# VITA-Group/LightGaussian

Hardware: NVIDIA H100
Metric: training views/sec at 3M Gaussians 1080p (higher is better)
Workload: dtype f32

## Files before the change

lightgaussian_b200/csrc/lgr_blend.cuh:

```cuda
#pragma once

namespace {

constexpr int BL_CH = 32;
constexpr int BL_STAGES = 4;
constexpr int BL_REC = 12;
constexpr int BL_THREADS = 288;
constexpr uint32_t BL_END = 0xffffffffu;
constexpr int BL_FLUSH = 16;
constexpr int BL_ROW = 33;

__device__ __forceinline__ void mbar_arrive(uint64_t* bar)
{
    asm volatile("mbarrier.arrive.shared::cta.b64 _, [%0];" ::"r"(smem_u32(bar)) : "memory");
}
__device__ __forceinline__ void mbar_wait_ring(uint64_t* bar, uint32_t parity)
{
    for (uint32_t spin = 0; !mbar_try_wait(bar, parity); ++spin)
        if (spin > (1u << 26)) {
            printf("lgrast: blend ring barrier timed out (block %d warp %d)\n", (int)blockIdx.x, (int)(threadIdx.x >> 5));
            __trap();
        }
}
template <int N>
// ... 31 lines not shown

constexpr int KB_ZERO_BYTES = 5760;

struct KbackZeroArgs {
    int P, nrest;
    const int* radii;
    const float* acc;
    int* idx;
    int* counter;
    float* d_xyz; float* d_dc; float* d_rest; float* d_scaling; float* d_rotation; float* d_opacity; float* dL_dmeans2D;
};

__device__ __forceinline__ void bulk_zero(float* dst, size_t floats, const void* zero_page)
{
    size_t bytes = floats * 4;
    char* p = reinterpret_cast<char*>(dst);
    while (bytes) {
        const uint32_t n = (uint32_t)(bytes < (size_t)KB_ZERO_BYTES ? bytes : (size_t)KB_ZERO_BYTES);
        bulk_s2g(p, zero_page, n);
        p += n;
        bytes -= n;
    }
}


__device__ __forceinline__ void tile_zero_rows(const KbackZeroArgs& z, int tile, int tiles, const void* zero_page)
{
    const int G = ((z.P + tiles - 1) / tiles + 3) & ~3;
    const long long first = (long long)tile * G;
    if (first >= z.P) return;
    const int n = (int)min((long long)G, z.P - first), nb = n & ~3;
    if (nb) {
        bulk_zero(z.d_rest + (size_t)first * z.nrest, (size_t)nb * z.nrest, zero_page);
        bulk_zero(z.d_dc + (size_t)first * 3, (size_t)nb * 3, zero_page);
        bulk_zero(z.d_xyz + (size_t)first * 3, (size_t)nb * 3, zero_page);
        bulk_zero(z.d_scaling + (size_t)first * 3, (size_t)nb * 3, zero_page);
        bulk_zero(z.d_rotation + (size_t)first * 4, (size_t)nb * 4, zero_page);
        bulk_zero(z.d_opacity + (size_t)first, (size_t)nb, zero_page);
        bulk_zero(z.dL_dmeans2D + (size_t)first * 3, (size_t)nb * 3, zero_page);
        bulk_commit();
    }
    for (long long i = first + nb; i < first + n; i++) {
        for (int k = 0; k < z.nrest; k++) z.d_rest[(size_t)i * z.nrest + k] = 0.f;
        for (int k = 0; k < 3; k++) {
            z.d_dc[(size_t)i * 3 + k] = 0.f; z.d_xyz[(size_t)i * 3 + k] = 0.f; z.d_scaling[(size_t)i * 3 + k] = 0.f; z.dL_dmeans2D[(size_t)i * 3 + k] = 0.f;
        }
        for (int k = 0; k < 4; k++) z.d_rotation[(size_t)i * 4 + k] = 0.f;
        z.d_opacity[(size_t)i] = 0.f;
    }
}

struct BlendRing {
    float rec[BL_STAGES][BL_CH * BL_REC];
    uint64_t full[BL_STAGES];
    uint64_t empty[BL_STAGES];
    uint32_t count[BL_STAGES];
    int live;
    unsigned tile_max;
};

__device__ __forceinline__ void ring_init(BlendRing& r, int consumers)
{
    if (threadIdx.x == 0) {
#pragma unroll
        for (int s = 0; s < BL_STAGES; s++) {
            mbar_init(&r.full[s], 1);
            mbar_init(&r.empty[s], consumers);
        }
        r.live = consumers;
        r.tile_max = 0;
        fence_mbar_init();
    }
    __syncthreads();
}

template <bool COUNT, bool STORE, bool PERM = false>
__global__ void __launch_bounds__(BL_THREADS)
blend_forward_ring_kernel(const uint2* __restrict__ ranges, const uint32_t* __restrict__ point_list, int W, int H, int tiles_x,
                          const float2* __restrict__ means2D, const float4* __restrict__ conic_opacity, const float4* __restrict__ rgb,
                          const float* __restrict__ bg, float* __restrict__ final_T, uint32_t* __restrict__ n_contrib,
                          float* __restrict__ out_color, int* __restrict__ count, float* __restrict__ rec_out, const int* __restrict__ header,
                          const uint32_t* __restrict__ perm = nullptr)
{
    if (header[HDR_OVERFLOW]) return;
    __shared__ __align__(128) BlendRing ring;
    const int warp = threadIdx.x >> 5, lane = threadIdx.x & 31;
    const int tile = blockIdx.x;
    const uint2 range = ranges[tile];
    ring_init(ring, 8);

    if (warp == 8) {
        for (uint32_t c = 0;; c++) {
            const int s = c % BL_STAGES;
            const uint32_t ph = (c / BL_STAGES) & 1u;
            mbar_wait_ring(&ring.empty[s], ph ^ 1u);
            if (STORE) {
                if (lane == 0) bulk_wait_read<BL_STAGES - 1>();
                __syncwarp();
            }
            const uint32_t pos0 = range.x + c * BL_CH;
            const int live = *reinterpret_cast<volatile int*>(&ring.live);
            if (pos0 >= range.y || live <= 0) {
                if (lane == 0) {
                    ring.count[s] = BL_END;
                    mbar_arrive(&ring.full[s]);
                }
                break;
            }
            const uint32_t n = min((uint32_t)BL_CH, range.y - pos0);
            if ((uint32_t)lane < n) {
                const uint32_t id = point_list[pos0 + lane];
                const float2 xy = means2D[id];
                const float4 co = conic_opacity[id];
                const float4 col = rgb[id];
                float4* r4 = reinterpret_cast<float4*>(&ring.rec[s][lane * BL_REC]);
                r4[0] = make_float4(xy.x, xy.y, co.x, co.y);
                r4[1] = make_float4(co.z, co.w, col.x, col.y);
                r4[2] = make_float4(col.z, __uint_as_float(id), PERM ? __uint_as_float(perm[pos0 + lane]) : 0.f, 0.f);
            }
            if (lane == 0) ring.count[s] = n;
            if (STORE) fence_async_smem();
            __syncwarp();
            if (lane == 0) {
                if (STORE) {
                    bulk_s2g(rec_out + (size_t)pos0 * BL_REC, &ring.rec[s][0], n * (uint32_t)(BL_REC * 4));
                    bulk_commit();
                }
                mbar_arrive(&ring.full[s]);
            }
        }
        if (STORE && lane == 0) bulk_wait_all();
        return;
    }

    const int tx = tile % tiles_x, ty = tile / tiles_x;
    const int sx0 = tx * LGR_TILE + (warp & 1) * 8, sy0 = ty * LGR_TILE + (warp >> 1) * 4;
    const int px = sx0 + (lane & 7), py = sy0 + (lane >> 3);
    const bool inside = px < W && py < H;
    float pxf = (float)px, pyf = (float)py;
    const float rx0 = (float)sx0, rx1 = (float)min(sx0 + 7, W - 1), ry0 = (float)sy0, ry1 = (float)min(sy0 + 3, H - 1);

    float T = inside ? 1.0f : -1.0f;
    float C0 = 0.f, C1 = 0.f, C2 = 0.f;
    uint32_t last = 0;
    bool warp_done = __all_sync(FULL, T < 0.f);
    if (warp_done && lane == 0) atomicSub(&ring.live, 1);

    for (uint32_t c = 0;; c++) {
        const int s = c % BL_STAGES;
        const uint32_t ph = (c / BL_STAGES) & 1u;
        mbar_wait_ring(&ring.full[s], ph);
        const uint32_t n = ring.count[s];
        if (n == BL_END) break;
        if (!warp_done) {
            const float* stage = &ring.rec[s][0];
            bool keep = false;
            if ((uint32_t)lane < n) {
                const float4 q0 = *reinterpret_cast<const float4*>(stage + lane * BL_REC);
                const float4 q1 = *reinterpret_cast<const float4*>(stage + lane * BL_REC + 4);
                keep = !subtile_cull2(q0.x, q0.y, q0.z, q0.w, q1.x, q1.y, rx0, rx1, ry0, ry1);
            }
            unsigned mask = __ballot_sync(FULL, keep);
            const uint32_t pos_base = c * BL_CH + 1u;
            while (mask) {
                const int j = __ffs(mask) - 1;
                mask &= mask - 1;
                const float* r = stage + j * BL_REC;
                const float4 q0 = *reinterpret_cast<const float4*>(r);
                const float4 q1 = *reinterpret_cast<const float4*>(r + 4);
                const float dx = LGR_SUB(q0.x, pxf), dy = LGR_SUB(q0.y, pyf);
                const float power = lgr::pair_power(dx, dy, q0.z, q0.w, q1.x);
                bool contrib = false;
                if (!(power > 0.0f)) {
                    const float alpha = fminf(0.99f, LGR_MUL(q1.y, expf(power)));
                    if (!(alpha < 1.0f / 255.0f)) {
                        const float test_T = LGR_MUL(T, LGR_SUB(1.0f, alpha));
                        if (test_T < 0.0001f) {
                            T = -fabsf(T);
                        } else {
                            const float b = r[8];
                            C0 = LGR_FMA(T, LGR_MUL(alpha, q1.z), C0);
                            C1 = LGR_FMA(T, LGR_MUL(alpha, q1.w), C1);
                            C2 = LGR_FMA(T, LGR_MUL(alpha, b), C2);
                            T = test_T;
                            last = pos_base + (uint32_t)j;
                            contrib = true;
                        }
                    }
                }
                if (COUNT) {
                    const unsigned cm = __ballot_sync(FULL, contrib);
                    if (cm != 0 && lane == 0) atomicAdd(&count[__float_as_uint(r[9])], __popc(cm));
                }
                if (__all_sync(FULL, T < 0.f)) break;
            }
            warp_done = __all_sync(FULL, T < 0.f);
            if (warp_done && lane == 0) atomicSub(&ring.live, 1);
        }
        __syncwarp();
        if (lane == 0) mbar_arrive(&ring.empty[s]);
    }
    if (inside) {
        const size_t pix = (size_t)py * W + px;
        const size_t plane = (size_t)H * W;
        const float Tf = fabsf(T);
        final_T[pix] = Tf;
        n_contrib[pix] = last;
        out_color[pix] = LGR_FMA(bg[0], Tf, C0);
        out_color[plane + pix] = LGR_FMA(bg[1], Tf, C1);
        out_color[2 * plane + pix] = LGR_FMA(bg[2], Tf, C2);
    }
}

struct BlendBackWarp {
    float w[BL_FLUSH][BL_ROW];
    float g[BL_FLUSH][BL_ROW];
    float mid[BL_FLUSH], mgx[BL_FLUSH], mgy[BL_FLUSH];
    float4 d[32];
};

struct BlendDetStage {
    float c[BL_STAGES][8][BL_CH * DET_ROW];
    uint32_t mask[BL_STAGES][8];
};

__host__ __device__ __forceinline__ size_t det_partial_offset(size_t Rn)
{
    return (Rn * 4 + 255) / 256 * 256 + (Rn * 48 + 255) / 256 * 256;
}
__host__ __device__ __forceinline__ size_t det_reached_offset(size_t Rn)
{
    return det_partial_offset(Rn) + (Rn * DET_ROW * 4 + 255) / 256 * 256;
}
__host__ __device__ __forceinline__ size_t det_ids_offset(size_t Rn)
{
    return det_reached_offset(Rn) + ((Rn + 31) / 32 * 4 + 255) / 256 * 256;
}

template <bool DET = false>
__device__ __forceinline__ void back_flush(const BlendBackWarp& bw, int nbuf, int lane, float ox, float oy, float* __restrict__ acc)
{
    __syncwarp();
    const int p = lane & 15, h = lane >> 4;
    float c0 = 0.f, c1 = 0.f, c2 = 0.f, s0 = 0.f, mx = 0.f, my = 0.f, mxx = 0.f, mxy = 0.f, myy = 0.f;
    const float* wr = &bw.w[p][16 * h];
    const float* gr = &bw.g[p][16 * h];
    const float4* dr = &bw.d[16 * h];
#pragma unroll
    for (int i = 0; i < 16; i++) {
        const float w = wr[i], g = gr[i];
        const float4 d = dr[i];
        const float xl = (float)(i & 7), yl = (float)(i >> 3);
        c0 = fmaf(w, d.x, c0);
        c1 = fmaf(w, d.y, c1);
        c2 = fmaf(w, d.z, c2);
        s0 += g;
        mx = fmaf(g, xl, mx);
        my = fmaf(g, yl, my);
        mxx = fmaf(g, xl * xl, mxx);
        mxy = fmaf(g, xl * yl, mxy);
        myy = fmaf(g, yl * yl, myy);
    }
    const float X = bw.mgx[p] - ox, Y = bw.mgy[p] - (oy + 2.0f * (float)h);
    float s1x = fmaf(X, s0, -mx), s1y = fmaf(Y, s0, -my);
    float s2xx = fmaf(X, fmaf(X, s0, -2.0f * mx), mxx);
    float s2xy = fmaf(X, fmaf(Y, s0, -my), fmaf(-Y, mx, mxy));
    float s2yy = fmaf(Y, fmaf(Y, s0, -2.0f * my), myy);
    c0 += __shfl_xor_sync(FULL, c0, 16);
    c1 += __shfl_xor_sync(FULL, c1, 16);
    c2 += __shfl_xor_sync(FULL, c2, 16);
    s0 += __shfl_xor_sync(FULL, s0, 16);
    s1x += __shfl_xor_sync(FULL, s1x, 16);
    s1y += __shfl_xor_sync(FULL, s1y, 16);
    s2xx += __shfl_xor_sync(FULL, s2xx, 16);
    s2xy += __shfl_xor_sync(FULL, s2xy, 16);
    s2yy += __shfl_xor_sync(FULL, s2yy, 16);
    if (DET && p < nbuf) {
        float* row = acc + __float_as_uint(bw.mid[p]) * DET_ROW;
        if (h == 0) {
            row[0] = c0; row[1] = c1; row[2] = c2; row[3] = s0; row[4] = s1x;
        } else {
            row[5] = s1y; row[6] = s2xx; row[7] = s2xy; row[8] = s2yy;
        }
    } else if (p < nbuf) {
        float* rec = acc + (size_t)__float_as_uint(bw.mid[p]) * ACC_STRIDE;
        if (h == 0) {
            red_add_v4(rec, c0, c1, c2, s0);
        } else {
            red_add_v4(rec + 4, s1x, s1y, s2xx, s2xy);
            atomicAdd(rec + 8, s2yy);
        }
    }
    __syncwarp();
}

constexpr size_t BL_DET_BYTES = (sizeof(BlendDetStage) + 127) / 128 * 128;

constexpr size_t blend_back_smem_bytes(bool zero_rows = false, bool det = false)
{
    return (sizeof(BlendRing) + 127) / 128 * 128 + (8 * sizeof(BlendBackWarp) + 127) / 128 * 128 + (det ? BL_DET_BYTES : 0) +
           (zero_rows ? (size_t)KB_ZERO_BYTES : 0);
}

template <bool DET = false>
__global__ void __launch_bounds__(BL_THREADS)
blend_backward_ring_kernel(const uint2* __restrict__ ranges, const char* __restrict__ binning_blob, const int* __restrict__ header, int W, int H,
                           int tiles_x, const float* __restrict__ bg, const float* __restrict__ final_T, const uint32_t* __restrict__ n_contrib,
                           const float* __restrict__ dL_dpix, float* __restrict__ acc, KbackZeroArgs zero)
{
    extern __shared__ __align__(128) unsigned char blend_dyn_smem[];
    BlendRing& ring = *reinterpret_cast<BlendRing*>(blend_dyn_smem);
    BlendBackWarp* warps = reinterpret_cast<BlendBackWarp*>(blend_dyn_smem + ((sizeof(BlendRing) + 127) / 128) * 128);
    unsigned char* behind_warps = reinterpret_cast<unsigned char*>(warps) + (8 * sizeof(BlendBackWarp) + 127) / 128 * 128;
    BlendDetStage* det = reinterpret_cast<BlendDetStage*>(behind_warps);
    const int warp = threadIdx.x >> 5, lane = threadIdx.x & 31;
    const int tile = blockIdx.x;
    const uint2 range = ranges[tile];
    float* zero_page = reinterpret_cast<float*>(behind_warps + (DET ? BL_DET_BYTES : 0));
    const bool zero_rows = zero.P > 0;
    if (zero_rows) {
        for (int k = threadIdx.x; k < KB_ZERO_BYTES / 4; k += BL_THREADS) zero_page[k] = 0.f;
        fence_async_smem();
    }
    ring_init(ring, 8);
    if (zero_rows && threadIdx.x == 8 * 32) tile_zero_rows(zero, tile, gridDim.x, zero_page);

    const int tx = tile % tiles_x, ty = tile / tiles_x;
    const int sx0 = tx * LGR_TILE + (warp & 1) * 8, sy0 = ty * LGR_TILE + (warp >> 1) * 4;
    const int px = sx0 + (lane & 7), py = sy0 + (lane >> 3);
    const bool inside = warp < 8 && px < W && py < H;
    const size_t pix = (size_t)py * W + px;
    const size_t plane = (size_t)H * W;
    const uint32_t last = inside ? n_contrib[pix] : 0u;
    const uint32_t warp_max = __reduce_max_sync(FULL, last);
    if (lane == 0 && warp_max) atomicMax(&ring.tile_max, warp_max);
    __syncthreads();
    const uint32_t tile_max = ring.tile_max;
    if (tile_max == 0 || (DET && header[HDR_DET] != 1)) {
        if (zero_rows && threadIdx.x == 8 * 32) bulk_wait_all();
        return;
    }
    const uint32_t nchunks = (tile_max + BL_CH - 1) / BL_CH;

    if (DET && warp == 8) {
        const size_t Rn = (size_t)max(header[HDR_CAPACITY], 1);
        const float* rec_in = reinterpret_cast<const float*>(binning_blob + (Rn * 4 + 255) / 256 * 256);
        float* partial = reinterpret_cast<float*>(const_cast<char*>(binning_blob) + det_partial_offset(Rn));
        uint32_t* reached = reinterpret_cast<uint32_t*>(const_cast<char*>(binning_blob) + det_reached_offset(Rn));
        for (uint32_t i = 0; i < nchunks + BL_STAGES; i++) {
            const int s = i % BL_STAGES;
            const uint32_t ph = (i / BL_STAGES) & 1u;
            if (i >= BL_STAGES) {
                mbar_wait_ring(&ring.empty[s], ph ^ 1u);
                const uint32_t b = nchunks - 1 - (i - BL_STAGES);
                const uint32_t n = min((uint32_t)BL_CH, tile_max - b * BL_CH);
                if ((uint32_t)lane < n) {
                    const uint32_t u = __float_as_uint(ring.rec[s][lane * BL_REC + 10]);
                    float v[DET_ROW];
#pragma unroll
                    for (int k = 0; k < DET_ROW; k++) v[k] = 0.f;
#pragma unroll
                    for (int w = 0; w < 8; w++) {
                        if ((det->mask[s][w] >> lane) & 1u) {
                            const float* c = &det->c[s][w][lane * DET_ROW];
#pragma unroll
                            for (int k = 0; k < DET_ROW; k++) v[k] += c[k];
                        }
                    }
                    if (u < Rn) {
#pragma unroll
                        for (int k = 0; k < DET_ROW; k++) partial[(size_t)u * DET_ROW + k] = v[k];
                        atomicOr(&reached[u >> 5], 1u << (u & 31));
                    }
                }
                __syncwarp();
            }
            if (i >= nchunks) continue;
            if (lane == 0) {
                if (i < BL_STAGES) mbar_wait_ring(&ring.empty[s], ph ^ 1u);
                const uint32_t b = nchunks - 1 - i;
                const uint32_t n = min((uint32_t)BL_CH, tile_max - b * BL_CH);
                const uint32_t bytes = n * (uint32_t)(BL_REC * 4);
                mbar_expect_tx(&ring.full[s], bytes);
                bulk_g2s(&ring.rec[s][0], rec_in + ((size_t)range.x + (size_t)b * BL_CH) * BL_REC, bytes, &ring.full[s]);
            }
            __syncwarp();
        }
        if (zero_rows && lane == 0) bulk_wait_all();
        return;
    }
    if (warp == 8) {
        if (lane == 0) {
            const size_t Rn = (size_t)max(header[HDR_CAPACITY], 1);
            const float* rec_in = reinterpret_cast<const float*>(binning_blob + (Rn * 4 + 255) / 256 * 256);
            for (uint32_t i = 0; i < nchunks; i++) {
                const uint32_t b = nchunks - 1 - i;
                const int s = i % BL_STAGES;
                const uint32_t ph = (i / BL_STAGES) & 1u;
                mbar_wait_ring(&ring.empty[s], ph ^ 1u);
                const uint32_t n = min((uint32_t)BL_CH, tile_max - b * BL_CH);
                const uint32_t bytes = n * (uint32_t)(BL_REC * 4);
                mbar_expect_tx(&ring.full[s], bytes);
                bulk_g2s(&ring.rec[s][0], rec_in + ((size_t)range.x + (size_t)b * BL_CH) * BL_REC, bytes, &ring.full[s]);
            }
            if (zero_rows) bulk_wait_all();
        }
        return;
    }

    BlendBackWarp& bw = warps[warp];
    float pxf = (float)px, pyf = (float)py;
    const float rx0 = (float)sx0, rx1 = (float)min(sx0 + 7, W - 1), ry0 = (float)sy0, ry1 = (float)min(sy0 + 3, H - 1);
    const float T_final = inside ? final_T[pix] : 0.f;
    float T = T_final;
    float d0 = 0.f, d1 = 0.f, d2 = 0.f;
    if (inside) {
        d0 = dL_dpix[pix];
        d1 = dL_dpix[plane + pix];
        d2 = dL_dpix[2 * plane + pix];
    }
    bw.d[lane] = make_float4(d0, d1, d2, 0.f);
    float D = T_final * (bg[0] * d0 + bg[1] * d1 + bg[2] * d2);
    int nbuf = 0;
    __syncwarp();

    for (uint32_t i = 0; i < nchunks; i++) {
        const uint32_t b = nchunks - 1 - i;
        const int s = i % BL_STAGES;
        const uint32_t ph = (i / BL_STAGES) & 1u;
        mbar_wait_ring(&ring.full[s], ph);
        uint32_t wrote = 0;
        float* parked = DET ? &det->c[s][warp][0] : acc;
        if (b * BL_CH < warp_max) {
            const float* stage = &ring.rec[s][0];
            const uint32_t n = min((uint32_t)BL_CH, tile_max - b * BL_CH);
            bool keep = false;
            if ((uint32_t)lane < n && b * BL_CH + (uint32_t)lane < warp_max) {
                const float4 q0 = *reinterpret_cast<const float4*>(stage + lane * BL_REC);
                const float4 q1 = *reinterpret_cast<const float4*>(stage + lane * BL_REC + 4);
                keep = !subtile_cull2(q0.x, q0.y, q0.z, q0.w, q1.x, q1.y, rx0, rx1, ry0, ry1);
            }
            unsigned mask = __ballot_sync(FULL, keep);
            while (mask) {
                const int j = 31 - __clz(mask);
                mask &= ~(1u << j);
                const float* r = stage + j * BL_REC;
                const float4 q0 = *reinterpret_cast<const float4*>(r);
                const float4 q1 = *reinterpret_cast<const float4*>(r + 4);
                const float2 q2 = *reinterpret_cast<const float2*>(r + 8);
                const float dx = q0.x - pxf, dy = q0.y - pyf;
                const float power = fmaf(-0.5f, fmaf(q0.z * dx, dx, q1.x * dy * dy), -q0.w * dx * dy);
                float G;
                asm("ex2.approx.ftz.f32 %0, %1;" : "=f"(G) : "f"(power * 1.4426950408889634f));
                float alpha = fminf(0.99f, q1.y * G);
                const bool on = (b * BL_CH + (uint32_t)j < last) && !(power > 0.0f) && !(alpha < 1.0f / 255.0f);
                if (!__any_sync(FULL, on)) continue;
                G = on ? G : 0.f;
                alpha = on ? alpha : 0.f;
                const float one_m_a = 1.0f - alpha;
                float rcp;
                asm("rcp.approx.ftz.f32 %0, %1;" : "=f"(rcp) : "f"(one_m_a));
                rcp = fmaf(rcp, fmaf(-one_m_a, rcp, 1.0f), rcp);
                T = T * rcp;
                const float cd = fmaf(q1.z, d0, fmaf(q1.w, d1, q2.x * d2));
                const float dL_dalpha = fmaf(T, cd, -rcp * D);
                const float w = alpha * T;
                D = fmaf(w, cd, D);
                bw.w[nbuf][lane] = w;
                bw.g[nbuf][lane] = G * dL_dalpha;
                if (lane == 0) {
                    bw.mid[nbuf] = DET ? __uint_as_float((uint32_t)j) : q2.y;
                    bw.mgx[nbuf] = q0.x;
                    bw.mgy[nbuf] = q0.y;
                }
                if (DET) wrote |= 1u << j;
                if (++nbuf == BL_FLUSH) {
                    back_flush<DET>(bw, nbuf, lane, rx0, ry0, parked);
                    nbuf = 0;
                }
            }
        }
        if (DET) {
            if (nbuf) back_flush<DET>(bw, nbuf, lane, rx0, ry0, parked);
            nbuf = 0;
            if (lane == 0) det->mask[s][warp] = wrote;
            __threadfence_block();
        }
        __syncwarp();
        if (lane == 0) mbar_arrive(&ring.empty[s]);
    }
    if (!DET && nbuf) back_flush(bw, nbuf, lane, rx0, ry0, acc);
}

__global__ void __launch_bounds__(256)
det_gather_kernel(int P, const uint32_t* __restrict__ tiles_kept, const unsigned long long* __restrict__ offsets,
                  const char* __restrict__ binning_blob, const int* __restrict__ header, float* __restrict__ acc)
{
    const int t = blockIdx.x * blockDim.x + threadIdx.x;
    if (t >= P) return;
    if (header[HDR_DET] != 1) {
        float4* rec = reinterpret_cast<float4*>(acc + (size_t)t * ACC_STRIDE);
        rec[0] = rec[1] = rec[2] = make_float4(__int_as_float(0x7fc00000), __int_as_float(0x7fc00000), __int_as_float(0x7fc00000), 0.f);
        return;
    }
    if (tiles_kept[t] == 0) {
        float4* rec = reinterpret_cast<float4*>(acc + (size_t)t * ACC_STRIDE);
        rec[0] = rec[1] = rec[2] = make_float4(0.f, 0.f, 0.f, 0.f);
    }
    const uint32_t end = (uint32_t)offsets[t], begin = t ? (uint32_t)offsets[t - 1] : 0u;
    if (end == begin) return;
    const size_t Rn = (size_t)max(header[HDR_CAPACITY], 1);
    const float* partial = reinterpret_cast<const float*>(binning_blob + det_partial_offset(Rn));
    const uint32_t* reached = reinterpret_cast<const uint32_t*>(binning_blob + det_reached_offset(Rn));
    const uint32_t* ids_unsorted = reinterpret_cast<const uint32_t*>(binning_blob + det_ids_offset(Rn));
    float v[DET_ROW];
#pragma unroll
    for (int q = 0; q < DET_ROW; q++) v[q] = 0.f;
    for (uint32_t u = begin; u < end; u++) {
        if (!((reached[u >> 5] >> (u & 31)) & 1u)) continue;
        const float* r = partial + (size_t)u * DET_ROW;
#pragma unroll
        for (int q = 0; q < DET_ROW; q++) v[q] += r[q];
    }
    float4* rec = reinterpret_cast<float4*>(acc + (size_t)ids_unsorted[begin] * ACC_STRIDE);
    rec[0] = make_float4(v[0], v[1], v[2], v[3]);
    rec[1] = make_float4(v[4], v[5], v[6], v[7]);
    rec[2] = make_float4(v[8], 0.f, 0.f, 0.f);
}

}
```

lightgaussian_b200/csrc/lgrast.cu:

```cuda
#include <cuda_runtime.h>
#include <cuda_fp16.h>
#include <cub/cub.cuh>
#include <thrust/iterator/transform_iterator.h>
#include <thrust/iterator/counting_iterator.h>
#include <cfloat>
#include <cmath>
#include <algorithm>
#include <atomic>
#include <cstdio>
#include <cstring>
#include <mutex>
#include <string>
#include <vector>

#include "../../include/lgrast.h"
#include "lgr_math.cuh"

namespace {

constexpr unsigned FULL = 0xffffffffu;
constexpr int LGR_SMS = 132;
constexpr int ACC_STRIDE = 12;
constexpr int DET_ROW = 9;

// ... 150 lines not shown
        g.iota = c.take<uint32_t>(P);
        g.offsets = c.take<unsigned long long>(P);
        size_t sort_bytes = 0, scan_bytes = 0;
        cub::DeviceRadixSort::SortPairs(nullptr, sort_bytes, (const uint32_t*)nullptr, (uint32_t*)nullptr, (const uint32_t*)nullptr,
                                        (uint32_t*)nullptr, (int)P, 0, 32);
        auto it = thrust::make_transform_iterator((const uint32_t*)nullptr, TilesTouchedOp{nullptr, nullptr});
        cub::DeviceScan::InclusiveSum(nullptr, scan_bytes, it, (unsigned long long*)nullptr, (int)P);
        g.cub_temp_bytes = sort_bytes > scan_bytes ? sort_bytes : scan_bytes;
        g.cub_temp = c.take<char>(g.cub_temp_bytes);
    }
    g.total = align_up(c.off, 256);
    return g;
}

struct ImageState {
    float* final_T;
    uint32_t* n_contrib;
    uint2* ranges;
    uint32_t* bin_M;
    uint32_t* bin_total;
    uint32_t* bin_base;
    size_t offs[3];
    size_t total;
};

ImageState carve_image(char* base, int W, int H, bool library_binning)
{
    ImageState s;
    const size_t N = (size_t)W * H;
    const size_t tiles = (size_t)((W + LGR_TILE - 1) / LGR_TILE) * ((H + LGR_TILE - 1) / LGR_TILE);
    Carver c(base);
    s.final_T = c.take<float>(N, &s.offs[0]);
    s.n_contrib = c.take<uint32_t>(N, &s.offs[1]);
    s.ranges = c.take<uint2>(tiles, &s.offs[2]);
    s.bin_M = s.bin_total = s.bin_base = nullptr;
    if (!library_binning) {
        const size_t pad = std::max((size_t)DS_BINS, (size_t)bin_pad((int)tiles));
        s.bin_M = c.take<uint32_t>((size_t)BIN_V * pad);
        s.bin_total = c.take<uint32_t>(pad);
        s.bin_base = c.take<uint32_t>(pad);
    }
    s.total = align_up(c.off, 256);
    return s;
}

inline int tile_key_bits(int W, int H)
{
    const uint32_t tiles = (uint32_t)((W + LGR_TILE - 1) / LGR_TILE) * ((H + LGR_TILE - 1) / LGR_TILE);
    int bits = 1;
    while ((1u << bits) < tiles) bits++;
    return bits;
}

struct BinningState {
    uint32_t* point_list;
    uint32_t* ids_unsorted;
    void* keys_unsorted;
    void* keys_sorted;
    char* cub_temp;
    size_t cub_temp_bytes;
    float* records;
    float* det_partial;
    uint32_t* det_reached;
    bool wide_keys;
    size_t offs[1];
    size_t total;
};

BinningState carve_binning(char* base, size_t R, int W, int H, bool library_binning, bool det = false)
{
    BinningState b;
    const int bits = tile_key_bits(W, H);
    b.wide_keys = bits > 16;
    const size_t Rn = R ? R : 1;
    Carver c(base);
    b.point_list = c.take<uint32_t>(Rn, &b.offs[0]);
    b.records = c.take<float>(Rn * 12);
    b.ids_unsorted = nullptr; b.keys_unsorted = b.keys_sorted = nullptr; b.cub_temp = nullptr; b.cub_temp_bytes = 0;
    b.det_partial = nullptr; b.det_reached = nullptr;
    if (!library_binning) {
        b.total = align_up(c.off, 256);
        return b;
    }
    if (det) {
        b.det_partial = c.take<float>(Rn * DET_ROW);
        b.det_reached = c.take<uint32_t>((Rn + 31) / 32);
    }
    b.ids_unsorted = c.take<uint32_t>(Rn);
    const size_t ksz = b.wide_keys ? 4 : 2;
    b.keys_unsorted = c.take<char>(Rn * ksz);
    b.keys_sorted = c.take<char>(Rn * ksz);
    size_t bytes = 0;
    if (b.wide_keys)
        cub::DeviceRadixSort::SortPairs(nullptr, bytes, (const uint32_t*)nullptr, (uint32_t*)nullptr, (const uint32_t*)nullptr,
                                        (uint32_t*)nullptr, (int)Rn, 0, bits);
    else
        cub::DeviceRadixSort::SortPairs(nullptr, bytes, (const uint16_t*)nullptr, (uint16_t*)nullptr, (const uint32_t*)nullptr,
                                        (uint32_t*)nullptr, (int)Rn, 0, bits);
    b.cub_temp_bytes = bytes;
    b.cub_temp = c.take<char>(bytes);
    b.total = align_up(c.off, 256);
    return b;
}

__device__ __forceinline__ bool subtile_cull(float gxp, float gyp, float4 co, float rx0, float rx1, float ry0, float ry1)
{
    const float A = co.x, B = co.y, Cc = co.z;
    const float t = 257.55f * co.w;
    if (t <= 1.0f) return true;
    if (!(A > 0.f && Cc > 0.f && A * Cc - B * B > 0.f)) return false;
    return lgr::rect_culled(0.5f * A, 0.5f * Cc, B, __fdividef(-B, A), __fdividef(-B, Cc), __logf(t), gxp - rx1, gxp - rx0, gyp - ry1,
                            gyp - ry0);
}

__device__ bool g_tile_cull_enabled = true;

__device__ __forceinline__ void tile_keep_mask(const lgr::Geom& geo, float4 co, int W, int H, unsigned long long& mask, uint32_t& kept)
{
    const int w = geo.rect.x1 - geo.rect.x0, h = geo.rect.y1 - geo.rect.y0;
    const int area = w * h;
    mask = ~0ull;
    kept = (uint32_t)area;
    if (area > 64) return;
    if (area < 64) mask = (1ull << area) - 1ull;
    if (!g_tile_cull_enabled) return;
    const float A = co.x, B = co.y, Cc = co.z;
    const float t = 257.55f * co.w;
    if (t <= 1.0f) {
        mask = 0ull;
        kept = 0;
// ... 817 lines not shown

    ImageState img = carve_image(nullptr, W, H, lib_bin);
    char* img_blob = image_alloc(image_user, img.total);
    if (!img_blob) { g_last_error = "image allocator returned NULL"; return LGR_ERR_ALLOC; }
    img = carve_image(img_blob, W, H, lib_bin);

    {
        PreprocessArgs a;
        a.P = P; a.D = v->sh_degree; a.M = M; a.W = W; a.H = H; a.gx = gx; a.gy = gy;
        a.fy = H / (2.0f * v->tan_fovy);
        a.fx = W / (2.0f * v->tan_fovx);
        a.tanx = v->tan_fovx; a.tany = v->tan_fovy; a.mod = v->scale_modifier;
        a.means3D = means3D; a.scales = scales; a.rotations = rotations; a.opacities = opacities; a.shs = shs;
        a.cov3D_precomp = cov3D_precomp; a.colors_precomp = colors_precomp;
        a.view = v->viewmatrix; a.proj = v->projmatrix; a.campos = v->campos; a.prefiltered = v->prefiltered;
        const int blocks = (P + 255) / 256;
        if (raw) {
            RawArgs ra = raw_args(a, gx, gy);
            ra.xyz = raw->xyz;
            ra.rest_stride = raw_rest_stride(raw, M);
            const LeafSource src = {raw->features_dc, raw->features_rest, raw->scaling, raw->rotation, raw->opacity};
            const size_t smem = raw_smem_bytes_stride(ra.rest_stride);
            LGR_CUDA_TRY(cudaFuncSetAttribute(preprocess_raw_kernel<LeafSource>, cudaFuncAttributeMaxDynamicSharedMemorySize, (int)smem));
            ProfScope ps(ST_PREPROCESS, stream);
            preprocess_raw_kernel<<<blocks, 256, smem, stream>>>(ra, src, radii, geo);
        } else if (vq) {
            RawArgs ra = raw_args(a, gx, gy);
            ra.xyz = vq->xyz;
            ra.rest_stride = (M - 1) * 3;
            const VqSource src = {vq->attr, vq->slot, static_cast<const __half*>(vq->codebook), vq->nonvq, vq->attr_half, vq->nonvq_half,
                                  vq->D, vq->Dp, M};
            const size_t smem = raw_smem_bytes_stride(ra.rest_stride);
            LGR_CUDA_TRY(cudaFuncSetAttribute(preprocess_raw_kernel<VqSource>, cudaFuncAttributeMaxDynamicSharedMemorySize, (int)smem));
            ProfScope ps(ST_PREPROCESS, stream);
            preprocess_raw_kernel<<<blocks, 256, smem, stream>>>(ra, src, radii, geo);
        } else {
            ProfScope ps(ST_PREPROCESS, stream);
            preprocess_kernel<<<blocks, 256, 0, stream>>>(a, radii, geo);
        }
        LGR_LAUNCH_CHECK("preprocess_kernel", debug, stream);
    }

    int R = 0, R_ref = 0;
    BinningState bin = {};
    const bool det = g_det != 0;
    int* host_hdr = t_pinned.get();

    auto launch_blend = [&]() -> int {
        if (count_mode) LGR_CUDA_TRY(cudaMemsetAsync(gaussians_count, 0, sizeof(int) * (size_t)P, stream));
        ProfScope ps(count_mode ? ST_BLEND_FWD_COUNT : ST_BLEND_FWD, stream);
        if (g_blend_mode == 0 && count_mode)
            blend_forward_ring_kernel<true, false><<<tiles, BL_THREADS, 0, stream>>>(img.ranges, bin.point_list, W, H, gx, geo.means2D, geo.conic_opacity,
                                                                                      geo.rgb, v->background, img.final_T, img.n_contrib, out_color,
                                                                                      gaussians_count, nullptr, geo.num_rendered);
        else if (g_blend_mode == 0 && det)
            blend_forward_ring_kernel<false, true, true><<<tiles, BL_THREADS, 0, stream>>>(img.ranges, bin.point_list, W, H, gx, geo.means2D,
                                                                                            geo.conic_opacity, geo.rgb, v->background, img.final_T,
                                                                                            img.n_contrib, out_color, nullptr, bin.records,
                                                                                            geo.num_rendered, reinterpret_cast<const uint32_t*>(bin.det_partial));
        else if (g_blend_mode == 0)
            blend_forward_ring_kernel<false, true><<<tiles, BL_THREADS, 0, stream>>>(img.ranges, bin.point_list, W, H, gx, geo.means2D, geo.conic_opacity,
                                                                                      geo.rgb, v->background, img.final_T, img.n_contrib, out_color,
                                                                                      nullptr, bin.records, geo.num_rendered);
        else if (count_mode)
            blend_forward_kernel<true><<<tiles, 256, 0, stream>>>(img.ranges, bin.point_list, W, H, gx, geo.means2D, geo.conic_opacity,
                                                                   geo.rgb, v->background, img.final_T, img.n_contrib, out_color,
                                                                   gaussians_count, geo.num_rendered);
        else
            blend_forward_kernel<false><<<tiles, 256, 0, stream>>>(img.ranges, bin.point_list, W, H, gx, geo.means2D, geo.conic_opacity,
                                                                    geo.rgb, v->background, img.final_T, img.n_contrib, out_color,
                                                                    nullptr, geo.num_rendered);
        LGR_LAUNCH_CHECK("blend_forward_kernel", debug, stream);
        return LGR_OK;
    };

    if (!lib_bin) {
        const int per_block = bin_per_block(P);
        const int tiles_pad = bin_pad(tiles);
        {
            ProfScope ps(ST_BIN_DSORT, stream);
            BinScanArgs sa;
            sa.M = img.bin_M; sa.V = BIN_V; sa.bins = DS_BINS; sa.bins_pad = DS_BINS; sa.bin_total = img.bin_total; sa.bin_base = img.bin_base;
            sa.header = geo.num_rendered; sa.ranges = nullptr; sa.capacity = 0;
            dsort_count_kernel<0, true><<<BIN_V, 256, 0, stream>>>(geo.depth_keys, P, per_block, img.bin_M, geo.num_rendered);
            bin_scan_kernel<false><<<DS_BINS / 32, SCAN_THREADS, 0, stream>>>(sa);
            dsort_scatter_kernel<0, true, false><<<BIN_V, DS_THREADS, 0, stream>>>(geo.depth_keys, nullptr, geo.depth_keys_sorted, geo.sorted_ids, img.bin_M,
                                                                           img.bin_base, P, per_block);
            dsort_count_kernel<DS_BITS, false><<<BIN_V, 256, 0, stream>>>(geo.depth_keys_sorted, P, per_block, img.bin_M, geo.num_rendered);
            bin_scan_kernel<false><<<DS_BINS / 32, SCAN_THREADS, 0, stream>>>(sa);
            dsort_scatter_kernel<DS_BITS, false, false><<<BIN_V, DS_THREADS, 0, stream>>>(geo.depth_keys_sorted, geo.sorted_ids, geo.depth_keys, geo.iota,
                                                                                  img.bin_M, img.bin_base, P, per_block);
            dsort_count_kernel<2 * DS_BITS, false><<<BIN_V, 256, 0, stream>>>(geo.depth_keys, P, per_block, img.bin_M, geo.num_rendered);
            bin_scan_kernel<false><<<DS_BINS / 32, SCAN_THREADS, 0, stream>>>(sa);
            dsort_scatter_kernel<2 * DS_BITS, false, true><<<BIN_V, DS_THREADS, 0, stream>>>(geo.depth_keys, geo.iota, nullptr, geo.sorted_ids, img.bin_M,
                                                                                      img.bin_base, P, per_block);
            g_launches.fetch_add(8, std::memory_order_relaxed);
            LGR_LAUNCH_CHECK("depth sort kernels", debug, stream);
        }
        const size_t tb_smem = sizeof(uint32_t) * (size_t)tiles_pad, ts_smem = tile_scatter_smem(tiles_pad);
        LGR_CUDA_TRY(cudaFuncSetAttribute(tile_count_kernel, cudaFuncAttributeMaxDynamicSharedMemorySize, (int)std::max(tb_smem, (size_t)48 * 1024)));
        LGR_CUDA_TRY(cudaFuncSetAttribute(tile_scatter_kernel, cudaFuncAttributeMaxDynamicSharedMemorySize, (int)std::max(ts_smem, (size_t)48 * 1024)));
        const bool exact = g_bin_mode == 1;
        size_t capacity = 0;
        if (!exact) {
            capacity = std::max(g_bin_hint.load(std::memory_order_relaxed), (size_t)4096);
            bin = carve_binning(nullptr, capacity, W, H, false);
            char* bin_blob = binning_alloc(binning_user, bin.total);
            if (!bin_blob) { g_last_error = "binning allocator returned NULL"; return LGR_ERR_ALLOC; }
            bin = carve_binning(bin_blob, capacity, W, H, false);
        }
        {
            ProfScope ps(ST_BIN_COUNT, stream);
            tile_count_kernel<<<BIN_V, TC_THREADS, tb_smem, stream>>>(geo.sorted_ids, geo.bin_rec, P, per_block, gx, tiles_pad, img.bin_M, geo.num_rendered);
            BinScanArgs sa;
            sa.M = img.bin_M; sa.V = BIN_V; sa.bins = tiles; sa.bins_pad = tiles_pad; sa.bin_total = img.bin_total; sa.bin_base = img.bin_base;
            sa.header = geo.num_rendered; sa.ranges = img.ranges;
// ... 96 lines not shown
                ProfScope ps(ST_RANGES, stream);
                ranges_kernel<uint32_t><<<(gx * gy + 255) / 256, 256, 0, stream>>>(R, gx * gy, (const uint32_t*)bin.keys_sorted, img.ranges);
            } else {
                {
                    ProfScope ps(ST_EMIT, stream);
                    emit_kernel<uint16_t><<<blocks, 256, 0, stream>>>(P, geo.sorted_ids, geo.offsets, geo.tiles_kept, geo.keep_mask, geo.means2D,
                                                                       radii, gx, gy, (uint16_t*)bin.keys_unsorted, bin.ids_unsorted);
                }
                LGR_LAUNCH_CHECK("emit_kernel", debug, stream);
                {
                    ProfScope ps(ST_TILE_SORT, stream);
                    if (det) {
                        const int st = det_tile_sort<uint16_t>(bin, R, bits, debug, stream);
                        if (st != LGR_OK) return st;
                    } else
                        LGR_CUDA_TRY(cub::DeviceRadixSort::SortPairs(bin.cub_temp, tmp, (const uint16_t*)bin.keys_unsorted,
                                                                      (uint16_t*)bin.keys_sorted, (const uint32_t*)bin.ids_unsorted,
                                                                      bin.point_list, R, 0, bits, stream));
                }
                ProfScope ps(ST_RANGES, stream);
                ranges_kernel<uint16_t><<<(gx * gy + 255) / 256, 256, 0, stream>>>(R, gx * gy, (const uint16_t*)bin.keys_sorted, img.ranges);
            }
            LGR_LAUNCH_CHECK("ranges_kernel", debug, stream);
        }
        const int st = launch_blend();
        if (st != LGR_OK) return st;
    }
    if (count_mode && P > 0) {
        ProfScope ps(ST_SCORE, stream);
        if (raw || vq) score_from_geom_kernel<<<(P + 255) / 256, 256, 0, stream>>>(P, gaussians_count, geo.conic_opacity, important_score);
        else score_kernel<<<(P + 255) / 256, 256, 0, stream>>>(P, gaussians_count, opacities, important_score);
        LGR_LAUNCH_CHECK("score_kernel", debug, stream);
    }
    (void)N;
    *num_rendered = R_ref;
    return LGR_OK;
}

int blend_backward_det(const GeometryState& geo, const ImageState& img, char* binning_blob, int P, int W, int H, const float* background,
                       const float* dL_dout_color, const KbackZeroArgs& zr, bool debug, cudaStream_t stream)
{
    const int gx = (W + LGR_TILE - 1) / LGR_TILE, gy = (H + LGR_TILE - 1) / LGR_TILE;
    {
        ProfScope ps(ST_BLEND_BWD, stream);
        const size_t bsmem = blend_back_smem_bytes(zr.P > 0, true);
        LGR_CUDA_TRY(cudaFuncSetAttribute(blend_backward_ring_kernel<true>, cudaFuncAttributeMaxDynamicSharedMemorySize,
                                          (int)blend_back_smem_bytes(true, true)));
        blend_backward_ring_kernel<true><<<gx * gy, BL_THREADS, bsmem, stream>>>(img.ranges, binning_blob, geo.num_rendered, W, H, gx, background,
                                                                                  img.final_T, img.n_contrib, dL_dout_color, geo.grad_acc, zr);
        LGR_LAUNCH_CHECK("blend_backward_ring_kernel<det>", debug, stream);
    }
    {
        ProfScope ps(ST_DET_GATHER, stream);
        det_gather_kernel<<<(P + 255) / 256, 256, 0, stream>>>(P, geo.tiles_kept, geo.offsets, binning_blob, geo.num_rendered, geo.grad_acc);
        LGR_LAUNCH_CHECK("det_gather_kernel", debug, stream);
    }
    return LGR_OK;
}

}

extern "C" {

int lgr_abi_version(void) { return LGR_ABI_VERSION; }
const char* lgr_last_error(void) { return g_last_error.c_str(); }
uint64_t lgr_launch_count(void) { return g_launches.load(); }

int lgr_set_blend_mode(int mode)
{
    if (mode != 0 && mode != 1) {
        g_last_error = "lgr_set_blend_mode: 0 = ring kernels (default), 1 = round-1 kernels";
        return LGR_ERR_INVALID_ARG;
    }
    g_blend_mode = mode;
    return LGR_OK;
}

int lgr_set_binning_mode(int mode)
{
    if (mode < 0 || mode > 2) {
        g_last_error = "lgr_set_binning_mode: 0 = hand-written kernels, estimated blob size, 1 = hand-written kernels, exact blob size, 2 = library sorts (default)";
        return LGR_ERR_INVALID_ARG;
    }
    g_bin_mode = mode;
    return LGR_OK;
}

int lgr_set_deterministic(int on)
{
    g_det = on != 0;
    return LGR_OK;
}

int lgr_set_kback_mode(int mode)
{
    if (mode < 0 || mode > 2) {
        g_last_error = "lgr_set_kback_mode: 0 = rows cleared inside the blend backward + compacted K7+K8 (default), 1 = dense K7+K8 kernel, 2 = separate zero-fill kernel + compacted K7+K8";
        return LGR_ERR_INVALID_ARG;
    }
    g_kback_mode = mode;
    return LGR_OK;
}

int lgr_set_vq_mode(int mode)
{
    if (mode != 0 && mode != 1) {
        g_last_error = "lgr_set_vq_mode: 0 = tensor-core coarse pass + exact FP32 rescore (default), 1 = FP32 kernel only";
// ... 1258 lines not shown
```

Baseline: 332.9.

## Reuse forward subtile cull masks in backward blend instead of recomputing

The forward ring kernel now records each warp's subtile-cull ballot mask per chunk into shared memory, and the producer warp streams these masks to a new global keep buffer. The backward kernel bulk-loads those masks alongside the records and uses them directly, dropping the per-chunk cull test and ballot. It also packs the backward staging buffers into one array with float4 metadata, and clears the processed bit with a bmsk instruction. The cost is extra global writes and reads for the mask buffer, a larger binning blob layout, and a drain loop at the end of the producer warp.

```diff
diff --git a/lightgaussian_b200/csrc/lgr_blend.cuh b/lightgaussian_b200/csrc/lgr_blend.cuh
--- a/lightgaussian_b200/csrc/lgr_blend.cuh
+++ b/lightgaussian_b200/csrc/lgr_blend.cuh
@@ -107,6 +107,7 @@
 
 struct BlendRing {
     float rec[BL_STAGES][BL_CH * BL_REC];
+    __align__(16) uint32_t keep[BL_STAGES][8];
     uint64_t full[BL_STAGES];
     uint64_t empty[BL_STAGES];
     uint32_t count[BL_STAGES];
@@ -134,8 +135,8 @@
 blend_forward_ring_kernel(const uint2* __restrict__ ranges, const uint32_t* __restrict__ point_list, int W, int H, int tiles_x,
                           const float2* __restrict__ means2D, const float4* __restrict__ conic_opacity, const float4* __restrict__ rgb,
                           const float* __restrict__ bg, float* __restrict__ final_T, uint32_t* __restrict__ n_contrib,
-                          float* __restrict__ out_color, int* __restrict__ count, float* __restrict__ rec_out, const int* __restrict__ header,
-                          const uint32_t* __restrict__ perm = nullptr)
+                          float* __restrict__ out_color, int* __restrict__ count, float* __restrict__ rec_out, uint32_t* __restrict__ keep_out,
+                          const int* __restrict__ header, const uint32_t* __restrict__ perm = nullptr)
 {
     if (header[HDR_OVERFLOW]) return;
     __shared__ __align__(128) BlendRing ring;
@@ -145,12 +146,14 @@
     ring_init(ring, 8);
 
     if (warp == 8) {
-        for (uint32_t c = 0;; c++) {
+        uint32_t c = 0;
+        for (;; c++) {
             const int s = c % BL_STAGES;
             const uint32_t ph = (c / BL_STAGES) & 1u;
             mbar_wait_ring(&ring.empty[s], ph ^ 1u);
             if (STORE) {
                 if (lane == 0) bulk_wait_read<BL_STAGES - 1>();
+                if (c >= BL_STAGES && lane < 8) keep_out[bin_keep_row(range.x, c - BL_STAGES, tile) * 8 + lane] = ring.keep[s][lane];
                 __syncwarp();
             }
             const uint32_t pos0 = range.x + c * BL_CH;
@@ -184,7 +187,13 @@
                 mbar_arrive(&ring.full[s]);
             }
         }
-        if (STORE && lane == 0) bulk_wait_all();
+        if (STORE) {
+            for (uint32_t k = c > BL_STAGES - 1 ? c - (BL_STAGES - 1) : 0; k < c; k++) {
+                mbar_wait_ring(&ring.empty[k % BL_STAGES], (k / BL_STAGES) & 1u);
+                if (lane < 8) keep_out[bin_keep_row(range.x, k, tile) * 8 + lane] = ring.keep[k % BL_STAGES][lane];
+            }
+            if (lane == 0) bulk_wait_all();
+        }
         return;
     }
 
@@ -216,6 +225,7 @@
                 keep = !subtile_cull2(q0.x, q0.y, q0.z, q0.w, q1.x, q1.y, rx0, rx1, ry0, ry1);
             }
             unsigned mask = __ballot_sync(FULL, keep);
+            if (STORE && lane == 0) ring.keep[s][warp] = mask;
             const uint32_t pos_base = c * BL_CH + 1u;
             while (mask) {
                 const int j = __ffs(mask) - 1;
@@ -268,9 +278,8 @@
 }
 
 struct BlendBackWarp {
-    float w[BL_FLUSH][BL_ROW];
-    float g[BL_FLUSH][BL_ROW];
-    float mid[BL_FLUSH], mgx[BL_FLUSH], mgy[BL_FLUSH];
+    float t[2 * BL_FLUSH * BL_ROW];
+    float4 meta[BL_FLUSH];
     float4 d[32];
 };
 
@@ -279,27 +288,14 @@
     uint32_t mask[BL_STAGES][8];
 };
 
-__host__ __device__ __forceinline__ size_t det_partial_offset(size_t Rn)
-{
-    return (Rn * 4 + 255) / 256 * 256 + (Rn * 48 + 255) / 256 * 256;
-}
-__host__ __device__ __forceinline__ size_t det_reached_offset(size_t Rn)
-{
-    return det_partial_offset(Rn) + (Rn * DET_ROW * 4 + 255) / 256 * 256;
-}
-__host__ __device__ __forceinline__ size_t det_ids_offset(size_t Rn)
-{
-    return det_reached_offset(Rn) + ((Rn + 31) / 32 * 4 + 255) / 256 * 256;
-}
-
 template <bool DET = false>
 __device__ __forceinline__ void back_flush(const BlendBackWarp& bw, int nbuf, int lane, float ox, float oy, float* __restrict__ acc)
 {
     __syncwarp();
     const int p = lane & 15, h = lane >> 4;
     float c0 = 0.f, c1 = 0.f, c2 = 0.f, s0 = 0.f, mx = 0.f, my = 0.f, mxx = 0.f, mxy = 0.f, myy = 0.f;
-    const float* wr = &bw.w[p][16 * h];
-    const float* gr = &bw.g[p][16 * h];
+    const float* wr = &bw.t[p * BL_ROW + 16 * h];
+    const float* gr = &bw.t[(BL_FLUSH + p) * BL_ROW + 16 * h];
     const float4* dr = &bw.d[16 * h];
 #pragma unroll
     for (int i = 0; i < 16; i++) {
@@ -316,7 +312,8 @@
         mxy = fmaf(g, xl * yl, mxy);
         myy = fmaf(g, yl * yl, myy);
     }
-    const float X = bw.mgx[p] - ox, Y = bw.mgy[p] - (oy + 2.0f * (float)h);
+    const float4 m = bw.meta[p];
+    const float X = m.x - ox, Y = m.y - (oy + 2.0f * (float)h);
     float s1x = fmaf(X, s0, -mx), s1y = fmaf(Y, s0, -my);
     float s2xx = fmaf(X, fmaf(X, s0, -2.0f * mx), mxx);
     float s2xy = fmaf(X, fmaf(Y, s0, -my), fmaf(-Y, mx, mxy));
@@ -331,14 +328,14 @@
     s2xy += __shfl_xor_sync(FULL, s2xy, 16);
     s2yy += __shfl_xor_sync(FULL, s2yy, 16);
     if (DET && p < nbuf) {
-        float* row = acc + __float_as_uint(bw.mid[p]) * DET_ROW;
+        float* row = acc + __float_as_uint(m.w) * DET_ROW;
         if (h == 0) {
             row[0] = c0; row[1] = c1; row[2] = c2; row[3] = s0; row[4] = s1x;
         } else {
             row[5] = s1y; row[6] = s2xx; row[7] = s2xy; row[8] = s2yy;
         }
     } else if (p < nbuf) {
-        float* rec = acc + (size_t)__float_as_uint(bw.mid[p]) * ACC_STRIDE;
+        float* rec = acc + (size_t)__float_as_uint(m.w) * ACC_STRIDE;
         if (h == 0) {
             red_add_v4(rec, c0, c1, c2, s0);
         } else {
@@ -355,6 +352,16 @@
 {
     return (sizeof(BlendRing) + 127) / 128 * 128 + (8 * sizeof(BlendBackWarp) + 127) / 128 * 128 + (det ? BL_DET_BYTES : 0) +
            (zero_rows ? (size_t)KB_ZERO_BYTES : 0);
+}
+
+__device__ __forceinline__ void back_load_chunk(BlendRing& r, int s, const float* rec_in, const uint32_t* keep_in, uint2 range, int tile,
+                                                uint32_t b, uint32_t tile_max)
+{
+    const uint32_t n = min((uint32_t)BL_CH, tile_max - b * BL_CH);
+    const uint32_t bytes = n * (uint32_t)(BL_REC * 4);
+    mbar_expect_tx(&r.full[s], bytes + (uint32_t)sizeof(r.keep[s]));
+    bulk_g2s(&r.rec[s][0], rec_in + ((size_t)range.x + (size_t)b * BL_CH) * BL_REC, bytes, &r.full[s]);
+    bulk_g2s(&r.keep[s][0], keep_in + bin_keep_row(range.x, b, tile) * 8, (uint32_t)sizeof(r.keep[s]), &r.full[s]);
 }
 
 template <bool DET = false>
@@ -399,9 +406,10 @@
 
     if (DET && warp == 8) {
         const size_t Rn = (size_t)max(header[HDR_CAPACITY], 1);
-        const float* rec_in = reinterpret_cast<const float*>(binning_blob + (Rn * 4 + 255) / 256 * 256);
-        float* partial = reinterpret_cast<float*>(const_cast<char*>(binning_blob) + det_partial_offset(Rn));
-        uint32_t* reached = reinterpret_cast<uint32_t*>(const_cast<char*>(binning_blob) + det_reached_offset(Rn));
+        const float* rec_in = reinterpret_cast<const float*>(binning_blob + bin_records_offset(Rn));
+        const uint32_t* keep_in = reinterpret_cast<const uint32_t*>(binning_blob + bin_keep_offset(Rn));
+        float* partial = reinterpret_cast<float*>(const_cast<char*>(binning_blob) + det_partial_offset(Rn, gridDim.x));
+        uint32_t* reached = reinterpret_cast<uint32_t*>(const_cast<char*>(binning_blob) + det_reached_offset(Rn, gridDim.x));
         for (uint32_t i = 0; i < nchunks + BL_STAGES; i++) {
             const int s = i % BL_STAGES;
             const uint32_t ph = (i / BL_STAGES) & 1u;
@@ -433,11 +441,7 @@
             if (i >= nchunks) continue;
             if (lane == 0) {
                 if (i < BL_STAGES) mbar_wait_ring(&ring.empty[s], ph ^ 1u);
-                const uint32_t b = nchunks - 1 - i;
-                const uint32_t n = min((uint32_t)BL_CH, tile_max - b * BL_CH);
-                const uint32_t bytes = n * (uint32_t)(BL_REC * 4);
-                mbar_expect_tx(&ring.full[s], bytes);
-                bulk_g2s(&ring.rec[s][0], rec_in + ((size_t)range.x + (size_t)b * BL_CH) * BL_REC, bytes, &ring.full[s]);
+                back_load_chunk(ring, s, rec_in, keep_in, range, tile, nchunks - 1 - i, tile_max);
             }
             __syncwarp();
         }
@@ -447,16 +451,13 @@
     if (warp == 8) {
         if (lane == 0) {
             const size_t Rn = (size_t)max(header[HDR_CAPACITY], 1);
-            const float* rec_in = reinterpret_cast<const float*>(binning_blob + (Rn * 4 + 255) / 256 * 256);
+            const float* rec_in = reinterpret_cast<const float*>(binning_blob + bin_records_offset(Rn));
+            const uint32_t* keep_in = reinterpret_cast<const uint32_t*>(binning_blob + bin_keep_offset(Rn));
             for (uint32_t i = 0; i < nchunks; i++) {
-                const uint32_t b = nchunks - 1 - i;
                 const int s = i % BL_STAGES;
                 const uint32_t ph = (i / BL_STAGES) & 1u;
                 mbar_wait_ring(&ring.empty[s], ph ^ 1u);
-                const uint32_t n = min((uint32_t)BL_CH, tile_max - b * BL_CH);
-                const uint32_t bytes = n * (uint32_t)(BL_REC * 4);
-                mbar_expect_tx(&ring.full[s], bytes);
-                bulk_g2s(&ring.rec[s][0], rec_in + ((size_t)range.x + (size_t)b * BL_CH) * BL_REC, bytes, &ring.full[s]);
+                back_load_chunk(ring, s, rec_in, keep_in, range, tile, nchunks - 1 - i, tile_max);
             }
             if (zero_rows) bulk_wait_all();
         }
@@ -465,7 +466,7 @@
 
     BlendBackWarp& bw = warps[warp];
     float pxf = (float)px, pyf = (float)py;
-    const float rx0 = (float)sx0, rx1 = (float)min(sx0 + 7, W - 1), ry0 = (float)sy0, ry1 = (float)min(sy0 + 3, H - 1);
+    const float rx0 = (float)sx0, ry0 = (float)sy0;
     const float T_final = inside ? final_T[pix] : 0.f;
     float T = T_final;
     float d0 = 0.f, d1 = 0.f, d2 = 0.f;
@@ -477,6 +478,7 @@
     bw.d[lane] = make_float4(d0, d1, d2, 0.f);
     float D = T_final * (bg[0] * d0 + bg[1] * d1 + bg[2] * d2);
     int nbuf = 0;
+    float* const col = &bw.t[lane];
     __syncwarp();
 
     for (uint32_t i = 0; i < nchunks; i++) {
@@ -488,17 +490,14 @@
         float* parked = DET ? &det->c[s][warp][0] : acc;
         if (b * BL_CH < warp_max) {
             const float* stage = &ring.rec[s][0];
-            const uint32_t n = min((uint32_t)BL_CH, tile_max - b * BL_CH);
-            bool keep = false;
-            if ((uint32_t)lane < n && b * BL_CH + (uint32_t)lane < warp_max) {
-                const float4 q0 = *reinterpret_cast<const float4*>(stage + lane * BL_REC);
-                const float4 q1 = *reinterpret_cast<const float4*>(stage + lane * BL_REC + 4);
-                keep = !subtile_cull2(q0.x, q0.y, q0.z, q0.w, q1.x, q1.y, rx0, rx1, ry0, ry1);
-            }
-            unsigned mask = __ballot_sync(FULL, keep);
+            const uint32_t ahead = warp_max - b * BL_CH;
+            unsigned mask = ring.keep[s][warp] & (ahead >= (uint32_t)BL_CH ? FULL : (1u << ahead) - 1u);
+            const int lim = (int)last - (int)(b * BL_CH);
             while (mask) {
                 const int j = 31 - __clz(mask);
-                mask &= ~(1u << j);
+                uint32_t below;
+                asm("bmsk.clamp.b32 %0, 0, %1;" : "=r"(below) : "r"(j));
+                mask &= below;
                 const float* r = stage + j * BL_REC;
                 const float4 q0 = *reinterpret_cast<const float4*>(r);
                 const float4 q1 = *reinterpret_cast<const float4*>(r + 4);
@@ -508,7 +507,7 @@
                 float G;
                 asm("ex2.approx.ftz.f32 %0, %1;" : "=f"(G) : "f"(power * 1.4426950408889634f));
                 float alpha = fminf(0.99f, q1.y * G);
-                const bool on = (b * BL_CH + (uint32_t)j < last) && !(power > 0.0f) && !(alpha < 1.0f / 255.0f);
+                const bool on = (j < lim) && !(power > 0.0f) && !(alpha < 1.0f / 255.0f);
                 if (!__any_sync(FULL, on)) continue;
                 G = on ? G : 0.f;
                 alpha = on ? alpha : 0.f;
@@ -521,16 +520,12 @@
                 const float dL_dalpha = fmaf(T, cd, -rcp * D);
                 const float w = alpha * T;
                 D = fmaf(w, cd, D);
-                bw.w[nbuf][lane] = w;
-                bw.g[nbuf][lane] = G * dL_dalpha;
-                if (lane == 0) {
-                    bw.mid[nbuf] = DET ? __uint_as_float((uint32_t)j) : q2.y;
-                    bw.mgx[nbuf] = q0.x;
-                    bw.mgy[nbuf] = q0.y;
-                }
+                col[nbuf * BL_ROW] = w;
+                col[(BL_FLUSH + nbuf) * BL_ROW] = G * dL_dalpha;
+                if (lane == 0) bw.meta[nbuf] = make_float4(q0.x, q0.y, q2.x, DET ? __uint_as_float((uint32_t)j) : q2.y);
                 if (DET) wrote |= 1u << j;
                 if (++nbuf == BL_FLUSH) {
-                    back_flush<DET>(bw, nbuf, lane, rx0, ry0, parked);
+                    back_flush<DET>(bw, BL_FLUSH, lane, rx0, ry0, parked);
                     nbuf = 0;
                 }
             }
@@ -548,7 +543,7 @@
 }
 
 __global__ void __launch_bounds__(256)
-det_gather_kernel(int P, const uint32_t* __restrict__ tiles_kept, const unsigned long long* __restrict__ offsets,
+det_gather_kernel(int P, int tiles, const uint32_t* __restrict__ tiles_kept, const unsigned long long* __restrict__ offsets,
                   const char* __restrict__ binning_blob, const int* __restrict__ header, float* __restrict__ acc)
 {
     const int t = blockIdx.x * blockDim.x + threadIdx.x;
@@ -565,9 +560,9 @@
     const uint32_t end = (uint32_t)offsets[t], begin = t ? (uint32_t)offsets[t - 1] : 0u;
     if (end == begin) return;
     const size_t Rn = (size_t)max(header[HDR_CAPACITY], 1);
-    const float* partial = reinterpret_cast<const float*>(binning_blob + det_partial_offset(Rn));
-    const uint32_t* reached = reinterpret_cast<const uint32_t*>(binning_blob + det_reached_offset(Rn));
-    const uint32_t* ids_unsorted = reinterpret_cast<const uint32_t*>(binning_blob + det_ids_offset(Rn));
+    const float* partial = reinterpret_cast<const float*>(binning_blob + det_partial_offset(Rn, tiles));
+    const uint32_t* reached = reinterpret_cast<const uint32_t*>(binning_blob + det_reached_offset(Rn, tiles));
+    const uint32_t* ids_unsorted = reinterpret_cast<const uint32_t*>(binning_blob + det_ids_offset(Rn, tiles));
     float v[DET_ROW];
 #pragma unroll
     for (int q = 0; q < DET_ROW; q++) v[q] = 0.f;
diff --git a/lightgaussian_b200/csrc/lgrast.cu b/lightgaussian_b200/csrc/lgrast.cu
--- a/lightgaussian_b200/csrc/lgrast.cu
+++ b/lightgaussian_b200/csrc/lgrast.cu
@@ -226,6 +226,23 @@
     return bits;
 }
 
+__host__ __device__ __forceinline__ size_t bin_records_offset(size_t Rn) { return (Rn * 4 + 255) / 256 * 256; }
+__host__ __device__ __forceinline__ size_t bin_keep_offset(size_t Rn) { return bin_records_offset(Rn) + (Rn * 48 + 255) / 256 * 256; }
+__host__ __device__ __forceinline__ size_t bin_keep_rows(size_t Rn, size_t tiles) { return (Rn + 31) / 32 + tiles; }
+__device__ __forceinline__ size_t bin_keep_row(uint32_t first, uint32_t chunk, int tile) { return (size_t)((first + chunk * 32u) / 32u) + tile; }
+__host__ __device__ __forceinline__ size_t det_partial_offset(size_t Rn, size_t tiles)
+{
+    return bin_keep_offset(Rn) + (bin_keep_rows(Rn, tiles) * 32 + 255) / 256 * 256;
+}
+__host__ __device__ __forceinline__ size_t det_reached_offset(size_t Rn, size_t tiles)
+{
+    return det_partial_offset(Rn, tiles) + (Rn * DET_ROW * 4 + 255) / 256 * 256;
+}
+__host__ __device__ __forceinline__ size_t det_ids_offset(size_t Rn, size_t tiles)
+{
+    return det_reached_offset(Rn, tiles) + ((Rn + 31) / 32 * 4 + 255) / 256 * 256;
+}
+
 struct BinningState {
     uint32_t* point_list;
     uint32_t* ids_unsorted;
@@ -234,6 +251,7 @@
     char* cub_temp;
     size_t cub_temp_bytes;
     float* records;
+    uint32_t* keep;
     float* det_partial;
     uint32_t* det_reached;
     bool wide_keys;
@@ -250,6 +268,8 @@
     Carver c(base);
     b.point_list = c.take<uint32_t>(Rn, &b.offs[0]);
     b.records = c.take<float>(Rn * 12);
+    const size_t tiles = (size_t)((W + LGR_TILE - 1) / LGR_TILE) * ((H + LGR_TILE - 1) / LGR_TILE);
+    b.keep = c.take<uint32_t>(bin_keep_rows(Rn, tiles) * 8);
     b.ids_unsorted = nullptr; b.keys_unsorted = b.keys_sorted = nullptr; b.cub_temp = nullptr; b.cub_temp_bytes = 0;
     b.det_partial = nullptr; b.det_reached = nullptr;
     if (!library_binning) {
@@ -1173,16 +1193,16 @@
         if (g_blend_mode == 0 && count_mode)
             blend_forward_ring_kernel<true, false><<<tiles, BL_THREADS, 0, stream>>>(img.ranges, bin.point_list, W, H, gx, geo.means2D, geo.conic_opacity,
                                                                                       geo.rgb, v->background, img.final_T, img.n_contrib, out_color,
-                                                                                      gaussians_count, nullptr, geo.num_rendered);
+                                                                                      gaussians_count, nullptr, nullptr, geo.num_rendered);
         else if (g_blend_mode == 0 && det)
             blend_forward_ring_kernel<false, true, true><<<tiles, BL_THREADS, 0, stream>>>(img.ranges, bin.point_list, W, H, gx, geo.means2D,
                                                                                             geo.conic_opacity, geo.rgb, v->background, img.final_T,
-                                                                                            img.n_contrib, out_color, nullptr, bin.records,
+                                                                                            img.n_contrib, out_color, nullptr, bin.records, bin.keep,
                                                                                             geo.num_rendered, reinterpret_cast<const uint32_t*>(bin.det_partial));
         else if (g_blend_mode == 0)
             blend_forward_ring_kernel<false, true><<<tiles, BL_THREADS, 0, stream>>>(img.ranges, bin.point_list, W, H, gx, geo.means2D, geo.conic_opacity,
                                                                                       geo.rgb, v->background, img.final_T, img.n_contrib, out_color,
-                                                                                      nullptr, bin.records, geo.num_rendered);
+                                                                                      nullptr, bin.records, bin.keep, geo.num_rendered);
         else if (count_mode)
             blend_forward_kernel<true><<<tiles, 256, 0, stream>>>(img.ranges, bin.point_list, W, H, gx, geo.means2D, geo.conic_opacity,
                                                                    geo.rgb, v->background, img.final_T, img.n_contrib, out_color,
@@ -1385,7 +1405,7 @@
     }
     {
         ProfScope ps(ST_DET_GATHER, stream);
-        det_gather_kernel<<<(P + 255) / 256, 256, 0, stream>>>(P, geo.tiles_kept, geo.offsets, binning_blob, geo.num_rendered, geo.grad_acc);
+        det_gather_kernel<<<(P + 255) / 256, 256, 0, stream>>>(P, gx * gy, geo.tiles_kept, geo.offsets, binning_blob, geo.num_rendered, geo.grad_acc);
         LGR_LAUNCH_CHECK("det_gather_kernel", debug, stream);
     }
     return LGR_OK;
```

Result: faster. 338.7, median of 6 (+1.7%).
